# shenwei356/bio

Hardware: AMD Instinct MI355X
Metric: Gbases/s hashed (k=21 ntHash + minimizer) (higher is better)
Workload: dtype u64

## Files before the change

bio_amd/csrc/kernels_pk.hpp:

```cpp
#pragma once
#include <utility>

#include "kernels_fast.hpp"

namespace bsk {

template <int... Is, class F>
__device__ __forceinline__ void pk_unroll_impl(std::integer_sequence<int, Is...>, F &&f) {
    (f(std::integral_constant<int, Is>{}), ...);
}
template <int N, class F>
__device__ __forceinline__ void pk_unroll(F &&f) {
    pk_unroll_impl(std::make_integer_sequence<int, N>{}, f);
}
template <int LO, int HI, class F>
__device__ __forceinline__ void pk_pick(u32 v, F &&f) {
    if constexpr (LO == HI) {
        f(std::integral_constant<int, LO>{});
    } else {
        constexpr int MID = (LO + HI) / 2;
        if (v <= (u32)MID) pk_pick<LO, MID>(v, f);
        else pk_pick<MID + 1, HI>(v, f);
    }
}

#ifndef BSK_PK_ROWS
#define BSK_PK_ROWS 58
#endif
struct PkLds {
    static constexpr int PR = BSK_PK_ROWS;
    static constexpr int ROW = 33;
    static constexpr int TAB = 0;
    static constexpr int TAB2 = 320;
    static constexpr int NHEADS = (32 * (PR - 1)) / 64 + 2;
    static constexpr int HEADS = 0;
    static constexpr int CTAB = 256;
    static constexpr int SH = 768;
    static constexpr int SP = SH + (PR + 1) * ROW * 8;
    static constexpr int TOTAL = (SP + (PR + 1) * ROW * 2 + 15) & ~15;
    static_assert(NHEADS * 8 <= CTAB && CTAB + 512 <= SH && TAB2 + 256 <= SH && TOTAL <= 20480, "PkLds");
};

struct PkTabs {
    u32x4 row;
    u32 at;
    __device__ __forceinline__ void init(int k, int lane, u32 tab = (u32)PkLds::TAB, u32 tab2 = (u32)PkLds::TAB2) {
        row = (u32x4){0, 0, 0, 0};
        at = 0xffffffffu;
        if (lane < 20) {
            const unsigned out = (unsigned)lane >> 2, in = (unsigned)lane & 3u;
            u64 f = seed_fwd_code(in);
            u64 r = rol64(seed_rev_code(in), (unsigned)(k - 1));
            if (out < 4) {
                f ^= rol64(seed_fwd_code(out), (unsigned)k);
                r ^= ror64(seed_rev_code(out), 1);
            }
            row = (u32x4){(u32)f, (u32)(f >> 32), (u32)r, (u32)(r >> 32)};
            at = tab + (u32)lane * 16u;
        } else if (lane >= 32 && lane < 48) {
            const unsigned c0 = (unsigned)lane & 3u, c1 = ((unsigned)lane >> 2) & 3u;
            const u64 f = rol64(seed_fwd_code(c0), 1) ^ seed_fwd_code(c1);
            const u64 r = ror64(rol64(seed_rev_code(c0), (unsigned)(k - 1)), 1) ^ rol64(seed_rev_code(c1), (unsigned)(k - 1));
            row = (u32x4){(u32)f, (u32)(f >> 32), (u32)r, (u32)(r >> 32)};
            at = tab2 + (u32)(lane - 32) * 16u;
        }
    }
    __device__ __forceinline__ void write(LDSQ char *ldsq) const {
        if (at != 0xffffffffu) *reinterpret_cast<LDSQ u32x4 *>(ldsq + at) = row;
        wave_sync_lds();
    }
};

template <int W>
struct PkCfg {
    static constexpr int XC = W > 12 ? 4 : W;
};

#define PKNW 16
typedef u32 u32x16 __attribute__((ext_vector_type(16)));
struct PkWords {
    u32x4 a, b, c, d;
};
__device__ __forceinline__ PkWords pk_load_words(const u32 *p) {
    PkWords r;
    asm volatile("global_load_dwordx4 %0, %4, off\n\tglobal_load_dwordx4 %1, %4, off offset:16\n\t"
                 "global_load_dwordx4 %2, %4, off offset:32\n\tglobal_load_dwordx4 %3, %4, off offset:48"
                 : "=&v"(r.a), "=&v"(r.b), "=&v"(r.c), "=&v"(r.d)
                 : "v"(p));
    return r;
}
__device__ __forceinline__ PkWords pk_load_words_n(const u32 *p, u32 nq) {
    PkWords r;
    asm volatile("global_load_dwordx4 %0, %4, off\n\t"
                 "s_cmp_lt_u32 %5, 3\n\ts_cbranch_scc1 .Lpkw_low%=\n\t"
                 "global_load_dwordx4 %1, %4, off offset:16\n\tglobal_load_dwordx4 %2, %4, off offset:32\n\t"
                 "s_cmp_lt_u32 %5, 4\n\ts_cbranch_scc1 .Lpkw_end%=\n\t"
                 "global_load_dwordx4 %3, %4, off offset:48\n\ts_branch .Lpkw_end%=\n"
                 ".Lpkw_low%=:\n\t"
                 "s_cmp_lt_u32 %5, 2\n\ts_cbranch_scc1 .Lpkw_end%=\n\t"
                 "global_load_dwordx4 %1, %4, off offset:16\n"
                 ".Lpkw_end%=:"
                 : "=&v"(r.a), "=&v"(r.b), "=&v"(r.c), "=&v"(r.d)
                 : "v"(p), "s"(nq)
                 : "scc");
    return r;
}
__device__ __forceinline__ u64 pk_load_u64(const u64 *p) {
    u64 r;
    asm volatile("global_load_dwordx2 %0, %1, off" : "=&v"(r) : "v"(p));
    return r;
}
__device__ __forceinline__ void pk_wait_loads(u64 &d0, u64 &d1) { asm volatile("s_waitcnt vmcnt(0)" : "+v"(d0), "+v"(d1)::"memory"); }
__device__ __forceinline__ void pk_wait_loads(PkWords &p) { asm volatile("s_waitcnt vmcnt(0)" : "+v"(p.a), "+v"(p.b), "+v"(p.c), "+v"(p.d)::"memory"); }
__device__ __forceinline__ void pk_ticket_async(u32 *ticket, u32 &t) {
    u64 ex;
    asm volatile("s_mov_b64 %1, exec\n\ts_mov_b64 exec, 1\n\tglobal_atomic_add %0, %2, %3, off sc0\n\ts_mov_b64 exec, %1"
                 : "+v"(t), "=&s"(ex)
                 : "v"(ticket), "v"(1u)
                 : "memory");
}
__device__ __forceinline__ void pk_wait_loads(PkWords &p, u64 &d0, u32 &f, u32 &t) {
    asm volatile("s_waitcnt vmcnt(0)" : "+v"(p.a), "+v"(p.b), "+v"(p.c), "+v"(p.d), "+v"(d0), "+v"(f), "+v"(t)::"memory");
}
__device__ __forceinline__ void pk_wait_loads(PkWords &p, u32 &f, u32 &t) {
    asm volatile("s_waitcnt vmcnt(0)" : "+v"(p.a), "+v"(p.b), "+v"(p.c), "+v"(p.d), "+v"(f), "+v"(t)::"memory");
}
__device__ __forceinline__ u32 pk_load_u8(const u8 *p) {
    u32 r;
    asm volatile("global_load_ubyte %0, %1, off" : "=&v"(r) : "v"(p));
    return r;
}
template <int W, bool LONG, class LY_ = PkLds, bool RINGM = false, bool SELM = false>
struct PkMin {
    typedef LY_ LY;
    const u32 *__restrict__ w;
    LDSQ char *lds;
    int k, lane;
    u32 nk;
    u32 fl, fh_, rl, rh_;
    u32 S[W];
    u64 H[W];
    u32 SB[W];
    u32 P, bm, tmin;
    u32 nsel;
    u32 slot, spare;
    u32 glo, gspan;
    u32 c8000;
    int sstep;
    u32 send;
    u32 in_lo, in_hi, out_lo, out_hi;
    u32x4 pw;
    u32x16 wr;
    static constexpr bool POS2 = !RINGM && !SELM;
    u32 i2;
    u32 nk_top;

    __device__ __forceinline__ void set_words(const PkWords &p) {
        wr = (u32x16){p.a.x, p.a.y, p.a.z, p.a.w, p.b.x, p.b.y, p.b.z, p.b.w, p.c.x, p.c.y, p.c.z, p.c.w, p.d.x, p.d.y, p.d.z, p.d.w};
    }
    __device__ __forceinline__ void word2(u32 i, u32 &lo, u32 &hi) const {
        const u32 iu = (u32)__builtin_amdgcn_readfirstlane((int)i);
        if (!LONG || iu + 1 < (u32)PKNW) {
            lo = wr[iu], hi = wr[iu + 1];
        } else {
            lo = w[iu], hi = w[iu + 1];
        }
    }
    __device__ __forceinline__ u32 word(u32 i) const {
        const u32 iu = (u32)__builtin_amdgcn_readfirstlane((int)i);
        if constexpr (RINGM) {
            if (iu < 4u) return iu == 0 ? pw.x : iu == 1 ? pw.y : iu == 2 ? pw.z : pw.w;
            return w[iu];
        }
        if (!LONG || iu < (u32)PKNW) return wr[iu];
        return w[iu];
    }
    __device__ __forceinline__ void load_block_words(u32 i0) {
        const u32 t0 = i0 + (u32)k - 1, p0 = i0 - 1;
        in_lo = w[t0 >> 4];
        in_hi = w[(t0 >> 4) + 1];
        out_lo = w[p0 >> 4];
        out_hi = w[(p0 >> 4) + 1];
    }
    __device__ __forceinline__ void load_block0_words() {
        const u32 t0 = (u32)k - 1;
        in_lo = word(t0 >> 4);
        in_hi = word((t0 >> 4) + 1);
        out_lo = word(0);
        out_hi = word(1);
    }
    __device__ __forceinline__ void roll(u32x4 x) {
        const u32 a = __builtin_amdgcn_alignbit(fl, fh_, 31), b = __builtin_amdgcn_alignbit(fh_, fl, 31);
        const u32 c = __builtin_amdgcn_alignbit(rh_, rl, 1), d = __builtin_amdgcn_alignbit(rl, rh_, 1);
        fl = a ^ x.x;
        fh_ = b ^ x.y;
        rl = c ^ x.z;
        rh_ = d ^ x.w;
    }
    __device__ __forceinline__ void roll2(u32x4 x) {
        const u32 a = __builtin_amdgcn_alignbit(fl, fh_, 30), b = __builtin_amdgcn_alignbit(fh_, fl, 30);
        const u32 c = __builtin_amdgcn_alignbit(rh_, rl, 2), d = __builtin_amdgcn_alignbit(rl, rh_, 2);
        fl = a ^ x.x;
        fh_ = b ^ x.y;
        rl = c ^ x.z;
        rh_ = d ^ x.w;
    }

    __device__ __forceinline__ void guard() {
        if constexpr (RINGM || SELM) return;
        const bool in = slot - glo <= gspan;
        slot = in ? slot : spare;
        sstep = in ? sstep : 0;
    }
    template <int IDX, int O>
    __device__ __forceinline__ void emit(u32 pbase) {
        if constexpr (!SELM) emit_staged<IDX, O>(pbase);
    }
    template <int IDX, int O>
    __device__ __forceinline__ void emit_staged(u32 pbase) {
        const u32 b = (bm >> IDX) & 1u;
        u32 pv;
        if constexpr (POS2) {
            (void)pbase;
            pv = SB[O];
        } else {
            asm("v_add3_u32 %0, %1, %2, %3" : "=v"(pv) : "v"(SB[O]), "s"(pbase), "n"(O));
        }
#if defined(PK_MASKST)
        {
            const u32 a0 = (u32)(uintptr_t)(lds + LY::SH) + slot, a1 = (u32)(uintptr_t)(lds + LY::SP) + (slot >> 2);
            u64 sv;
            asm volatile("v_cmp_ne_u32_e32 vcc, 0, %1\n\ts_and_saveexec_b64 %0, vcc\n\tds_write_b64 %2, %3\n\tds_write_b16 %4, %5\n\ts_mov_b64 exec, %0"
                         : "=&s"(sv) : "v"(b), "v"(a0), "v"(H[O]), "v"(a1), "v"(pv) : "vcc", "memory");
        }
#elif defined(PK_NOPOS)
        *reinterpret_cast<LDSQ u64 *>(lds + LY::SH + slot) = H[O];
#ifdef PK_STRMASK
        asm volatile("" ::"v"(pv));
#endif
#elif !defined(PK_NOSTAGE)
        *reinterpret_cast<LDSQ u64 *>(lds + LY::SH + slot) = H[O];
        *reinterpret_cast<LDSQ u16 *>(lds + LY::SP + (slot >> 2)) = (u16)pv;
#else
        asm volatile("" ::"v"(H[O]), "v"(pv), "v"(slot));
#endif
        asm("v_mad_i32_i24 %0, %1, %2, %0" : "+v"(slot) : "v"(b), "v"(sstep));
        if constexpr (RINGM) slot = slot == send ? (u32)lane * 8u : slot;
    }

    template <bool FIRST, bool RAG, int PAR>
    __device__ __forceinline__ void block(u32 i0, u32 okbit, bool suffix) {
        static_assert(!POS2, "POS2 (k_minimizer_pk): i2 is advanced by run()");
        const u32 t0 = i0 + (u32)k - 1, p0 = FIRST ? 0u : i0 - 1u;
        steps<FIRST, RAG, PAR>(2u * t0, 2u * p0, i0, okbit);
        if (suffix) suffix_pass();
        tail<FIRST, PAR>(i0);
    }

    template <bool FIRST, bool RAG, int PAR>
    __device__ __forceinline__ void steps(u32 t2, u32 p2, u32 i0, u32 okbit) {
        constexpr int CB = PAR * 16, PB = (1 - PAR) * 16;
        constexpr int XC = PkCfg<W>::XC;
        constexpr int O2 = PAR ? 0 : 2 * W;
        u32 in_lo, in_hi, out_lo, out_hi;
        if constexpr (RINGM) {
            in_lo = this->in_lo, in_hi = this->in_hi, out_lo = this->out_lo, out_hi = this->out_hi;
            load_block_words(i0 + (u32)W);
        } else {
            word2(t2 >> 5, in_lo, in_hi);
            word2(p2 >> 5, out_lo, out_hi);
        }
        const u32 cinb = __builtin_amdgcn_alignbit(in_hi, in_lo, t2 & 31u);
        u32 coutb;
        if (FIRST) coutb = out_lo << 2;
        else coutb = __builtin_amdgcn_alignbit(out_hi, out_lo, p2 & 31u);
        const u32 E = (cinb & 0x33333333u) | ((coutb & 0x33333333u) << 2);
        const u32 O = ((cinb >> 2) & 0x33333333u) | (coutb & 0xCCCCCCCCu);
        const u32 E4 = E << 4, O4 = O << 4;
        u32x4 xs[W];
        auto fetch = [&](int o0) {
#pragma unroll
            for (int o = o0; o < o0 + XC && o < W; ++o) {
                const int j = o >> 1;
                const u32 src = (j & 1) ? ((o & 1) ? O : E) : ((o & 1) ? O4 : E4);
                u32 a;
                switch (j >> 1) {
                    case 0: asm("v_and_b32_sdwa %0, %1, %2 dst_sel:DWORD dst_unused:UNUSED_PAD src0_sel:BYTE_0 src1_sel:DWORD" : "=v"(a) : "v"(src), "s"(0xF0u)); break;
                    case 1: asm("v_and_b32_sdwa %0, %1, %2 dst_sel:DWORD dst_unused:UNUSED_PAD src0_sel:BYTE_1 src1_sel:DWORD" : "=v"(a) : "v"(src), "s"(0xF0u)); break;
                    case 2: asm("v_and_b32_sdwa %0, %1, %2 dst_sel:DWORD dst_unused:UNUSED_PAD src0_sel:BYTE_2 src1_sel:DWORD" : "=v"(a) : "v"(src), "s"(0xF0u)); break;
                    default: asm("v_and_b32_sdwa %0, %1, %2 dst_sel:DWORD dst_unused:UNUSED_PAD src0_sel:BYTE_3 src1_sel:DWORD" : "=v"(a) : "v"(src), "s"(0xF0u)); break;
                }
                if (FIRST && o == 0) a = 0x100u | (a & 0x30u);
#ifndef PK_NOTAB
                xs[o] = *reinterpret_cast<LDSQ const u32x4 *>(lds + LY::TAB + a);
#else
                xs[o] = (u32x4){a, a ^ E, a + O, a ^ cinb};
#endif
            }
        };
        fetch(0);
        if (XC < W) fetch(XC);
        u32 pbase = 0;
        if constexpr (!POS2) pbase = (u32)__builtin_amdgcn_readfirstlane((int)(i0 - (u32)W));
        if (!FIRST) guard();
        u32 vb = 0;
        if (RAG && !FIRST) {
            const int left = (int)nk - (int)i0;
            const u32 nv = (u32)(left < 0 ? 0 : left > W ? W : left);
            vb = (1u << nv) - 1u;
        }
        constexpr bool CUTB = RAG && !FIRST;
        u32 live = (u32)W;
        if constexpr (CUTB) {
            const u32 left = nk_top - i0;
            live = (u32)__builtin_amdgcn_readfirstlane((int)(left < (u32)W ? left : (u32)W));
        }
        pk_unroll<W>([&](auto oc) {
            constexpr int o = decltype(oc)::value;
            if (XC < W && o && o % XC == 0 && o + XC < W) {
                __builtin_amdgcn_sched_barrier(0);
                fetch(o + XC);
            }
            if constexpr (CUTB) {
                this->template emit<PB + o, o>(pbase);
                if (o != 0 && (u32)o >= live) return;
            }
            roll(xs[o]);
            if constexpr (!CUTB) {
                if (!FIRST) this->template emit<PB + o, o>(pbase);
            }
            const lmask rev = lt64(rl, rh_, fl, fh_);
            const u32 hl = sel(rev, rl, fl), hh = sel(rev, rh_, fh_);
            if constexpr (POS2) {
                lmask co;
                asm("v_addc_co_u32_e64 %0, %1, %2, %3, %4" : "=v"(SB[o]), "=s"(co) : "n"(O2 + 2 * o), "v"(i2), "s"(rev));
            } else {
                asm("v_cndmask_b32_e64 %0, 0, %1, %2" : "=v"(SB[o]) : "v"(c8000), "s"(rev));
            }
            H[o] = ((u64)hh << 32) | hl;
            u32 pk;
            asm("v_and_or_b32 %0, %1, %2, %3" : "=v"(pk) : "v"(hh), "s"(0xffffffe0u), "n"(CB + o));
            if (o == 0) {
                P = pk;
            } else {
#ifndef PK_NOTIE
                const u32 d = pk ^ P;
                tmin = tmin < d ? tmin : d;
#endif
                P = P < pk ? P : pk;
            }
            if (!FIRST || o == W - 1) {
                u32 m = P;
                if constexpr (o != W - 1) {
#ifndef PK_NOTIE
                    const u32 d = P ^ S[o + 1];
                    tmin = tmin < d ? tmin : d;
#endif
                    m = P < S[o + 1] ? P : S[o + 1];
                }
                u32 one = 1u;
                if (FIRST) one = okbit;
                else if (RAG) one = (vb >> o) & 1u;
                bm |= one << (m & 31u);
            }
            S[o] = pk;
        });
    }

    __device__ __forceinline__ void suffix_pass() {
#pragma unroll
        for (int q = W - 2; q >= 1; --q) {
#ifndef PK_NOTIE
            const u32 d = S[q] ^ S[q + 1];
            tmin = tmin < d ? tmin : d;
#endif
            S[q] = S[q] < S[q + 1] ? S[q] : S[q + 1];
        }
    }

    template <bool FIRST, int PAR>
    __device__ __forceinline__ void tail(u32 i0) {
        constexpr int PB = (1 - PAR) * 16;
        if constexpr (SELM) {
            if (!FIRST) {
                const u32 wsel = (bm >> PB) & ((1u << W) - 1u);
                *reinterpret_cast<LDSQ u32 *>(lds + LY::MASK + (i0 / (u32)W - 1u) * 256u + (u32)lane * 4u) = wsel;
                nsel += (u32)__builtin_popcount(wsel);
            }
        }
        if (!FIRST) asm("v_and_b32_e32 %0, %1, %0" : "+v"(bm) : "n"(PAR ? 0xffff0000u : 0x0000ffffu));
    }

    template <int PAR, int O>
    __device__ __forceinline__ void drain_from(u32 pbase, u32 live) {
        if constexpr (O < W) {
            if (O == 0 || (u32)O < live) {
                this->template emit<PAR * 16 + O, O>(pbase);
                drain_from<PAR, O + 1>(pbase, live);
            }
        }
    }

    template <int PAR>
    __device__ __forceinline__ void drain(u32 i0, u32 live = (u32)W) {
        if constexpr (SELM) {
            const u32 wsel = (bm >> (PAR * 16)) & ((1u << W) - 1u);
            *reinterpret_cast<LDSQ u32 *>(lds + LY::MASK + (i0 / (u32)W) * 256u + (u32)lane * 4u) = wsel;
            nsel += (u32)__builtin_popcount(wsel);
            return;
        }
        const u32 pbase = (u32)__builtin_amdgcn_readfirstlane((int)i0);
        guard();
        drain_from<PAR, 0>(pbase, live);
    }

    __device__ __forceinline__ void begin(u32 slot0, int step, u32 col8) {
        fl = fh_ = rl = rh_ = 0;
        bm = 0;
        nsel = 0;
        nk_top = 0xffffffffu;
        c8000 = 0x8000u;
        asm volatile("" : "+v"(c8000));
        tmin = 0xffffffffu;
        slot = slot0;
        sstep = step;
        if constexpr (RINGM) {
            (void)col8;
            spare = glo = gspan = 0;
            send = (u32)(LY::ROWS * LY::ROW * 8) + (u32)lane * 8u;
        } else {
            spare = (u32)(LY::PR * LY::ROW * 8) + col8;
            send = 0;
            constexpr u32 RB = (u32)(LY::ROW * 8);
            glo = step < 0 ? col8 + (u32)(W - 1) * RB : col8;
            gspan = (u32)(LY::PR - W) * RB + (step < 0 ? 0u : RB);
        }
        if constexpr (RINGM) load_block0_words();
        for (int t0 = 0; t0 < k - 1; t0 += 16) {
            const u32 word = this->word((u32)t0 >> 4);
            const int nb = (k - 1 - t0) < 16 ? (k - 1 - t0) : 16;
            int j = 0;
            for (; j + 8 <= nb; j += 8) {
                const u32 sub = word >> (2 * j);
                const u32x4 x0 = *reinterpret_cast<LDSQ const u32x4 *>(lds + LY::TAB2 + ((sub & 0xf) << 4));
                const u32x4 x1 = *reinterpret_cast<LDSQ const u32x4 *>(lds + LY::TAB2 + (sub & 0xf0));
                const u32x4 x2 = *reinterpret_cast<LDSQ const u32x4 *>(lds + LY::TAB2 + ((sub & 0xf00) >> 4));
                const u32x4 x3 = *reinterpret_cast<LDSQ const u32x4 *>(lds + LY::TAB2 + ((sub & 0xf000) >> 8));
                roll2(x0);
                roll2(x1);
                roll2(x2);
                roll2(x3);
            }
            for (; j + 2 <= nb; j += 2) roll2(*reinterpret_cast<LDSQ const u32x4 *>(lds + LY::TAB2 + (((word >> (2 * j)) & 0xf) << 4)));
            for (; j < nb; ++j) roll(*reinterpret_cast<LDSQ const u32x4 *>(lds + LY::TAB + 256 + (((word >> (2 * j)) & 3) << 4)));
        }
    }

    static constexpr bool CARRY = !SELM;
    __device__ __forceinline__ void advance(u32 &i0, u32 &t2, u32 &p2) const {
        if constexpr (CARRY) {
            t2 += 2u * W, p2 += 2u * W;
            asm volatile("" : "+s"(t2), "+s"(p2));
            i0 = (p2 >> 1) + 1u;
        } else {
            i0 += W;
            t2 = 2u * (i0 + (u32)k - 1u), p2 = 2u * (i0 - 1u);
        }
    }

    __device__ __forceinline__ void run(u32 nk_max, bool ok, u32 nk_min, u32 slot0, int step, u32 col8) {
        begin(slot0, step, col8);
        nk_top = nk_max;
        if constexpr (POS2) i2 = (u32)(-2 * W);
        steps<true, false, 0>(2u * ((u32)k - 1u), 0u, 0u, ok ? 1u : 0u);
        if (nk_max <= (u32)W) {
            drain<0>(0);
            return;
        }
        suffix_pass();
        u32 i0 = W;
        u32 t2 = 2u * ((u32)W + (u32)k - 1u), p2 = 2u * ((u32)W - 1u);
        if constexpr (CARRY) asm volatile("" : "+s"(t2), "+s"(p2));
        const int lim = 2 * ((int)__builtin_amdgcn_readfirstlane((int)(nk_min < 0x8000u ? nk_min : 0x8000u)) - 2 * W - 1);
        while ((int)p2 < lim) {
            if constexpr (POS2) asm("v_add_u32_e32 %0, %1, %0" : "+v"(i2) : "n"(4 * W));
            steps<false, false, 1>(t2, p2, i0, 1u);
            suffix_pass();
            tail<false, 1>(i0);
            advance(i0, t2, p2);
            steps<false, false, 0>(t2, p2, i0, 1u);
            suffix_pass();
            tail<false, 0>(i0);
            advance(i0, t2, p2);
        }
        int last_par;
        for (;;) {
            if constexpr (POS2) asm("v_add_u32_e32 %0, %1, %0" : "+v"(i2) : "n"(4 * W));
            steps<false, true, 1>(t2, p2, i0, 1u);
            tail<false, 1>(i0);
            advance(i0, t2, p2);
            last_par = 1;
            if (i0 >= nk_max) break;
            suffix_pass();
            steps<false, true, 0>(t2, p2, i0, 1u);
            tail<false, 0>(i0);
            advance(i0, t2, p2);
            last_par = 0;
            if (i0 >= nk_max) break;
            suffix_pass();
        }
        const u32 left = nk_max - (i0 - (u32)W);
        const u32 live = (u32)__builtin_amdgcn_readfirstlane((int)(left < (u32)W ? left : (u32)W));
        if (last_par) drain<1>(i0 - W, live);
        else drain<0>(i0 - W, live);
    }
};

template <int U, class LY = PkLds, bool POS2 = false, bool TAILR = false>
__device__ __forceinline__ void pk_copyout(char *lds, int lane, u32 cnt, u32 excl, u32 T, u64 base, const KArgs &a) {
    constexpr int NH = LY::NHEADS;
    u64 *s_heads = reinterpret_cast<u64 *>(lds + LY::HEADS);
    u64 *s_tab64 = reinterpret_cast<u64 *>(lds + LY::CTAB);
    const u64 nzmask = __builtin_amdgcn_ballot_w64(cnt > 0);
    if (lane < NH) s_heads[lane] = 0;
    wave_sync_lds();
    if (cnt > 0) {
        constexpr int RB = LY::ROW * 8;
        const int col8 = (lane & 31) * 8;
        const int S = lane < 32 ? RB : -RB;
        const int A = lane < 32 ? col8 - (int)excl * RB : col8 + ((int)(LY::PR - 1) + (int)excl) * RB;
        const u32 rk = __builtin_amdgcn_mbcnt_hi((u32)(nzmask >> 32), __builtin_amdgcn_mbcnt_lo((u32)nzmask, 0));
        s_tab64[rk] = ((u64)(u32)S << 32) | (u32)A;
        if (excl) atomicOr(&s_heads[(excl - 1u) >> 6], 1ULL << ((excl - 1u) & 63u));
    }
    wave_sync_lds();
    const u64 hw = lane < NH ? s_heads[lane] : 0ULL;
    const u32 hw_lo = (u32)hw, hw_hi = (u32)(hw >> 32);
    u32 heads_before = 0;
    const char *sh = lds + LY::SH, *sp = lds + LY::SP;
    u64 *const gh = a.hash + base;
    u32 *const gp = a.pos + base;
    auto trip = [&](u32 t0, auto rows, auto check) {
        constexpr int R = decltype(rows)::value;
        constexpr bool CHECK = decltype(check)::value;
        u32 rank[R];
#pragma unroll
        for (int j = 0; j < R; ++j) {
            const u32 c = (t0 >> 6) + j;
            const u32 mlo = (u32)__builtin_amdgcn_readlane((int)hw_lo, (int)c), mhi = (u32)__builtin_amdgcn_readlane((int)hw_hi, (int)c);
            rank[j] = (__builtin_amdgcn_mbcnt_hi(mhi, __builtin_amdgcn_mbcnt_lo(mlo, 0u)) << 3) + (heads_before << 3);
            heads_before += (u32)__builtin_popcountll(((u64)mhi << 32) | mlo);
        }
        u64 ent[U];
#pragma unroll
        for (int j = 0; j < R; ++j) ent[j] = *reinterpret_cast<const u64 *>(reinterpret_cast<const char *>(s_tab64) + rank[j]);
#pragma unroll
        for (int j = R; j < U; ++j) ent[j] = ent[R - 1];
        if constexpr (U == 8) {
            __builtin_amdgcn_sched_barrier(0);
            asm volatile("" ::"v"(ent[0]), "v"(ent[1]), "v"(ent[2]), "v"(ent[3]), "v"(ent[4]), "v"(ent[5]), "v"(ent[6]), "v"(ent[7]));
            __builtin_amdgcn_sched_barrier(0);
        }
        u64 hv[U];
        u32 pv[U];
#pragma unroll
        for (int j = 0; j < R; ++j) {
            const u32 t = t0 + 64 * j + lane;
            const int off = __mul24((int)t, (int)(u32)(ent[j] >> 32)) + (int)(u32)ent[j];
            const u32 so = (!CHECK || (TAILR && j < R - 1) || t < T) ? (u32)off : 0u;
            hv[j] = *reinterpret_cast<const u64 *>(sh + so);
            if constexpr (POS2) pv[j] = *reinterpret_cast<const u16 *>(sp + (so >> 2));
            else pv[j] = (u32)(int)*reinterpret_cast<const short *>(sp + (so >> 2));
        }
#pragma unroll
        for (int j = R; j < U; ++j) hv[j] = hv[R - 1], pv[j] = pv[R - 1];
        if constexpr (U == 8) {
            __builtin_amdgcn_sched_barrier(0);
            asm volatile("" ::"v"(hv[0]), "v"(hv[1]), "v"(hv[2]), "v"(hv[3]), "v"(hv[4]), "v"(hv[5]), "v"(hv[6]), "v"(hv[7]), "v"(pv[0]), "v"(pv[1]),
                         "v"(pv[2]), "v"(pv[3]), "v"(pv[4]), "v"(pv[5]), "v"(pv[6]), "v"(pv[7]));
            __builtin_amdgcn_sched_barrier(0);
        }
#pragma unroll
        for (int j = 0; j < R; ++j) {
            const u32 t = t0 + 64 * j + lane;
#ifdef PK_NOSTORE
            asm volatile("" ::"v"(hv[j]), "v"(pv[j]));
#else
            if (!CHECK || (TAILR && j < R - 1) || t < T) {
#ifndef PK_NOHASHST
                __builtin_nontemporal_store(hv[j], &gh[t]);
#else
                asm volatile("" ::"v"(hv[j]));
#endif
#ifndef PK_NOPOSST
                __builtin_nontemporal_store(POS2 ? __builtin_amdgcn_alignbit(pv[j], pv[j], 1) : pv[j] & 0x80007fffu, &gp[t]);
#else
                asm volatile("" ::"v"(pv[j]));
#endif
            }
#endif
        }
    };
    u32 t0 = 0;
    for (; t0 + 64 * U <= T; t0 += 64 * U) trip(t0, std::integral_constant<int, U>{}, std::false_type{});
    if (t0 < T) {
        if constexpr (TAILR) {
            const u32 nr = (u32)__builtin_amdgcn_readfirstlane((int)((T - t0 + 63u) >> 6));
            pk_pick<1, U>(nr, [&](auto rc) { trip(t0, rc, std::true_type{}); });
        } else {
            trip(t0, std::integral_constant<int, U>{}, std::true_type{});
        }
    }
    wave_sync_lds();
}

#ifndef PK_TICKET
#define PK_TICKET 8u
#endif
template <int W, bool LONG, bool UNI = false>
__global__ __launch_bounds__(64, 2) void k_minimizer_pk(KArgs a) {
    static_assert(!(UNI && LONG), "k_minimizer_pk: the fixed-length form keeps the whole read in registers");
    typedef PkLds LY;
    __shared__ __attribute__((aligned(16))) char lds[LY::TOTAL];
    LDSQ char *const ldsq = (LDSQ char *)lds;
    const int lane = lane_id();
    PkTabs tabs;
    tabs.init(a.k, lane);
#ifdef PK_STAGGER
    for (u32 i = (((blockIdx.x * 2654435761u) >> 24) * (u32)PK_STAGGER) >> 8; i; --i) __builtin_amdgcn_s_sleep(32);
#endif
    const u64 slab = (u64)64 * BSK_FAST_CAP;
    const u32 col8 = (u32)(lane & 31) * 8u;
    constexpr u32 RB = (u32)(LY::ROW * 8);
    const u32 top = (u32)(LY::PR - 1) * RB + col8;
    u64 d_n1 = 0, d_cur = 0;
    PkWords pw_cur = {{0, 0, 0, 0}, {0, 0, 0, 0}, {0, 0, 0, 0}, {0, 0, 0, 0}};
    bool have = false;
    const u32 lseg = a.fixcap / a.list_grid;
    u32 lcur = 0;
    const u32 tku = a.tk ? a.tk : PK_TICKET;
    const u32 t0s = a.tk_small ? a.tk_t0 : 0xffffffffu, u0s = a.tk_small ? a.tk_t0 * tku : 0xffffffffu;
    const u32 tsm = a.tk_small ? a.tk_small : tku;
    auto ticket_unit = [&](u32 t) { return t < t0s ? t * tku : u0s + (t - t0s) * tsm; };
    auto ticket_end = [&](u32 first) { return first + (first < u0s ? tku : tsm); };
    const u32 uL = a.uniform_len;
    const u32 unk = (UNI && uL >= (u32)a.circ_ext && (uL - (u32)a.circ_ext) + 1u >= (u32)a.k + (u32)W) ? uL - (u32)a.k + 1u : 0u;
    const u32 unq = a.uni_stride / 4u + 1u < 4u ? a.uni_stride / 4u + 1u : 4u;
    const bool ahead = tku >= 3u;
    u32 tv = 0;
    u32 nt = ~0u;
    for (u32 unit = ticket_unit(next_ticket(a.ticket, lane)), uend = ticket_end(unit); unit < a.nunits; ++unit, ({
             if (unit == uend) {
                 unit = ahead ? nt : ticket_unit(next_ticket(a.ticket, lane));
                 uend = ticket_end(unit);
             }
         })) {
        const u64 r = (u64)unit * 64 + lane;
        const u64 u2 = (!ahead || unit + 2u < uend) ? (u64)unit + 2u : (u64)nt + (unit + 2u - uend);
        const bool nxt = unit + 1 != uend ? unit + 1 < a.nunits : ahead && nt < a.nunits;
        const bool ask = ahead && unit + 3u == uend;
        const u64 rmax = a.n - 1;
        if constexpr (UNI) {
            if (!have) {
                pw_cur = pk_load_words_n(a.words + (r < rmax ? r : rmax) * (u64)a.uni_stride, unq);
                pk_wait_loads(pw_cur);
            }
        } else if (!have) {
            d_cur = pk_load_u64(a.desc + (r < rmax ? r : rmax));
            d_n1 = pk_load_u64(a.desc + (r + 64 < rmax ? r + 64 : rmax));
            pk_wait_loads(d_cur, d_n1);
            pw_cur = pk_load_words(a.words + (d_cur >> 24));
            pk_wait_loads(pw_cur);
        }
        PkWords pw_n1;
        u64 d_n2 = 0;
        if constexpr (UNI) {
            const u64 r1 = ((!ahead || unit + 1u < uend) ? (u64)unit + 1u : (u64)nt) * 64 + lane;
            pw_n1 = pk_load_words_n(a.words + (r1 < rmax ? r1 : rmax) * (u64)a.uni_stride, unq);
        } else {
            pw_n1 = pk_load_words(a.words + (d_n1 >> 24));
            const u64 r2 = u2 * 64 + lane;
            d_n2 = pk_load_u64(a.desc + (r2 < rmax ? r2 : rmax));
        }
        u32 rfl = pk_load_u8(a.rflags ? a.rflags + (r < rmax ? r : rmax) : reinterpret_cast<const u8 *>(a.desc));
        if (ask) pk_ticket_async(a.ticket, tv);
        const u64 d = d_cur;
        const PkWords pw = pw_cur;
        u64 off, ro;
        bool ok;
        u32 nk, nk_max, nk_min;
        if constexpr (UNI) {
            off = 0;
            ro = r;
            ok = r < a.n && unk != 0u;
            nk = nk_max = nk_min = unk;
        } else {
            const u64 L = desc_len(a, d);
            off = d >> 24;
            ro = out_index(a, r, d);
            ok = r < a.n && L >= (u64)a.circ_ext && (L - (u64)a.circ_ext) + 1 >= (u64)a.k + (u64)W;
            nk = ok ? (u32)(L - a.k + 1) : 0u;
            nk_max = wave_max_u32(nk);
            nk_min = ~wave_max_u32(~(ok ? nk : 0xffffffffu));
        }
        u32 cnt = 0, tmin_lane = 0xffffffffu;
        if (nk_max) {
            tabs.write(ldsq);
            PkMin<W, LONG> pm;
            pm.w = a.words + off;
            pm.set_words(pw);
            pm.lds = ldsq;
            pm.k = a.k;
            pm.lane = lane;
            pm.nk = nk;
            const u32 spare = (u32)LY::PR * RB + col8;
            pm.run(nk_max, ok, nk_min, !ok ? spare : lane < 32 ? col8 : top, !ok ? 0 : lane < 32 ? (int)RB : -(int)RB, col8);
            if (ok) cnt = (lane < 32 ? pm.slot - col8 : top - pm.slot) / RB;
            tmin_lane = pm.tmin;
        }
        if constexpr (UNI) pk_wait_loads(pw_n1, rfl, tv);
        else pk_wait_loads(pw_n1, d_n2, rfl, tv);
        if (ask) nt = ticket_unit((u32)__builtin_amdgcn_readfirstlane((int)tv));
        d_cur = d_n1;
        pw_cur = pw_n1;
        d_n1 = d_n2;
        have = nxt;
        const u32 cnt_pair = cnt + (u32)__builtin_amdgcn_ds_bpermute((lane ^ 32) * 4, (int)cnt);
        u64 bad = __builtin_amdgcn_ballot_w64(cnt_pair >= (u32)LY::PR);
        u64 tied = __builtin_amdgcn_ballot_w64(ok && tmin_lane < 32u);
#if defined(PK_NOSTAGE) || defined(PK_NOTIE) || defined(PK_NOTAB) || defined(PK_NOCOPY) || defined(PK_NOSTORE) || defined(PK_NOFB)
        bad = 0;
        tied = 0;
#endif
        const u64 redo = bad | tied;
        if (redo) {
            list_append(a, a.rlist, lseg, lcur, redo, lane, r);
            if ((redo >> lane) & 1) cnt = 0;
        }
        const u32 incl = wave_incl_scan_u32(cnt, lane);
        const u32 excl = incl - cnt;
        const u32 T = wave_bcast_u32(incl, 63);
        const u64 base = (u64)unit * slab;
#ifndef PK_NOCOPY
#ifndef PK_CU
#define PK_CU 8
#endif
        if (T) pk_copyout<PK_CU, LY, PkMin<W, LONG>::POS2, true>(lds, lane, cnt, excl, T, base, a);
#endif
        if (r < a.n) {
            if (!((redo >> lane) & 1)) a.refs[ro] = ((base + excl) << 24) | cnt;
            u8 sbyte = ok ? BSK_ST_OK : BSK_ST_SHORT;
            if (ok && a.rflags) sbyte |= (u8)rfl;
            a.status[ro] = sbyte;
        }
    }
    list_close(a.rlist, lseg, lcur, lane);
}

#ifdef BSK_IMPL_PK
#ifndef BSK_PK_WS
#define BSK_PK_WS(X) X(2) X(3) X(4) X(5) X(6) X(7) X(8) X(9) X(10) X(11) X(12) X(13)
#endif
bool pk_minimizer_supported(int w) { return w >= 2 && w <= 13; }
u32 pk_minimizer_short_bases() { return 16u * (PKNW - 1); }
int pk_minimizer_blocks_per_cu(int w) {
    int nb = 0;
    hipError_t e = hipErrorInvalidValue;
    switch (w) {
#define X(WW) \
    case WW: e = hipOccupancyMaxActiveBlocksPerMultiprocessor(&nb, k_minimizer_pk<WW, false>, 64, 0); break;
        BSK_PK_WS(X)
#undef X
        default: break;
    }
    if (e != hipSuccess || nb < 1) {
        (void)hipGetLastError();
        nb = 1;
    }
    return nb;
}
void pk_minimizer_list_launch(int w, int grid, hipStream_t stream, const KArgs &a) {
    switch (w) {
#define X(WW) \
    case WW: hipLaunchKernelGGL((k_minimizer_dense<WW, true>), dim3(grid), dim3(64), 0, stream, a); break;
        BSK_PK_WS(X)
#undef X
        default: break;
    }
}
bool pk_minimizer_uniform(bool long_reads, const KArgs &a) { return !long_reads && a.uni_stride && a.uniform_len && !a.cls_hi && !a.binned && !a.subset; }
void pk_minimizer_launch(int w, bool long_reads, int grid, hipStream_t stream, const KArgs &a) {
    const bool uni = pk_minimizer_uniform(long_reads, a);
    switch (w) {
#define X(WW)                                                                                               \
    case WW:                                                                                                \
        if (long_reads) {                                                                                   \
            hipLaunchKernelGGL((k_minimizer_pk<WW, true>), dim3(grid), dim3(64), 0, stream, a);             \
        } else if (uni) {                                                                                   \
            hipLaunchKernelGGL((k_minimizer_pk<WW, false, true>), dim3(grid), dim3(64), 0, stream, a);      \
        } else {                                                                                            \
            hipLaunchKernelGGL((k_minimizer_pk<WW, false>), dim3(grid), dim3(64), 0, stream, a);            \
        }                                                                                                   \
        hipLaunchKernelGGL((k_minimizer_dense<WW, true>), dim3(grid), dim3(64), 0, stream, a);              \
        break;
        BSK_PK_WS(X)
#undef X
        default: break;
    }
}
#endif

}
```

bio_amd/csrc/kernels_ring.hpp:

```cpp
#pragma once
#include "kernels_pk.hpp"
#pragma clang diagnostic ignored "-Winline-asm"

namespace bsk {

typedef u32 u32x3 __attribute__((ext_vector_type(3)));
#ifdef RG_B96
typedef u32x3 u32x3_lds __attribute__((aligned(16)));
#else
typedef u32x3 u32x3_lds __attribute__((aligned(4)));
#endif

#ifndef BSK_RING_WAVES
#define BSK_RING_WAVES 3
#endif
#ifndef BSK_RING_NQ
#define BSK_RING_NQ (BSK_RING_WAVES >= 3 ? 3 : 4)
#endif
#ifndef BSK_RING_EVERY
#define BSK_RING_EVERY 1
#endif
#ifndef BSK_RING_FIRST
#define BSK_RING_FIRST 4
#endif
// ... 282 lines not shown
#else
        asm volatile("" ::"v"(HL[O]), "v"(HH[O]), "v"(pv), "v"(at));
#endif
        asm("v_lshl_add_u32 %0, %1, 28, %0" : "+v"(phase) : "v"(b));
    }

    template <bool FIRST, bool RAG, int PAR>
    __device__ __forceinline__ void block(u32 i0, u32 okbit, bool suffix) {
        constexpr int CB = PAR * 16, PB = (1 - PAR) * 16;
        constexpr int XC = RgCfg<W>::XC;
        const u32 t0 = i0 + (u32)k - 1, p0 = FIRST ? 0u : i0 - 1u;
        u32 in_lo, in_hi, out_lo, out_hi;
        this->template word2<PAR>(t0 >> 4, true, in_lo, in_hi);
        this->template word2<PAR>(p0 >> 4, false, out_lo, out_hi);
        const u32 cinb = __builtin_amdgcn_alignbit(in_hi, in_lo, (t0 & 15) * 2);
        u32 coutb;
        if (FIRST) coutb = out_lo << 2;
        else coutb = __builtin_amdgcn_alignbit(out_hi, out_lo, (p0 & 15) * 2);
        const u32 E = (cinb & 0x33333333u) | ((coutb & 0x33333333u) << 2);
        const u32 O = ((cinb >> 2) & 0x33333333u) | (coutb & 0xCCCCCCCCu);
        const u32 E4 = E << 4, O4 = O << 4;
        u32x4 xs[W];
        auto fetch = [&](int o0) {
#pragma unroll
            for (int o = o0; o < o0 + XC && o < W; ++o) {
                const int j = o >> 1;
                const u32 src = (j & 1) ? ((o & 1) ? O : E) : ((o & 1) ? O4 : E4);
                u32 a;
                switch (j >> 1) {
                    case 0: asm("v_and_b32_sdwa %0, %1, %2 dst_sel:DWORD dst_unused:UNUSED_PAD src0_sel:BYTE_0 src1_sel:DWORD" : "=v"(a) : "v"(src), "s"(0xF0u)); break;
                    case 1: asm("v_and_b32_sdwa %0, %1, %2 dst_sel:DWORD dst_unused:UNUSED_PAD src0_sel:BYTE_1 src1_sel:DWORD" : "=v"(a) : "v"(src), "s"(0xF0u)); break;
                    case 2: asm("v_and_b32_sdwa %0, %1, %2 dst_sel:DWORD dst_unused:UNUSED_PAD src0_sel:BYTE_2 src1_sel:DWORD" : "=v"(a) : "v"(src), "s"(0xF0u)); break;
                    default: asm("v_and_b32_sdwa %0, %1, %2 dst_sel:DWORD dst_unused:UNUSED_PAD src0_sel:BYTE_3 src1_sel:DWORD" : "=v"(a) : "v"(src), "s"(0xF0u)); break;
                }
                if (FIRST && o == 0) a = 0x100u | (a & 0x30u);
                xs[o] = *reinterpret_cast<LDSQ const u32x4 *>(lds + LY::TAB + a);
            }
        };
        fetch(0);
        if (XC < W) fetch(XC);
        u32 pbase = 2u * (i0 - (u32)W);
        asm volatile("" : "+v"(pbase));
        u32 vb = 0;
        if (RAG && !FIRST) {
            const int left = (int)nk - (int)i0;
            const u32 nv = (u32)(left < 0 ? 0 : left > W ? W : left);
            vb = (1u << nv) - 1u;
        }
        pk_unroll<W>([&](auto oc) {
            constexpr int o = decltype(oc)::value;
            if (XC < W && o && o % XC == 0 && o + XC < W) {
                __builtin_amdgcn_sched_barrier(0);
                fetch(o + XC);
            }
            roll(xs[o]);
            const lmask rev = lt64(rl, rh_, fl, fh_);
            if (!FIRST) this->template emit<PB + o, o>(pbase);
            const u32 hl = sel(rev, rl, fl), hh = sel(rev, rh_, fh_);
            HL[o] = hl;
            HH[o] = hh;
            RV[o] = rev;
            u32 pk;
            asm("v_and_or_b32 %0, %1, %2, %3" : "=v"(pk) : "v"(hh), "s"(0xffffffe0u), "n"(CB + o));
            if (o == 0) {
                P = pk;
            } else {
#ifndef RG_NOTIE
                const u32 d = pk ^ P;
                tmin = tmin < d ? tmin : d;
#endif
                P = P < pk ? P : pk;
            }
            if (!FIRST || o == W - 1) {
                u32 m = P;
                if constexpr (o != W - 1) {
#ifndef RG_NOTIE
                    const u32 d = P ^ S[o + 1];
                    tmin = tmin < d ? tmin : d;
#endif
                    m = P < S[o + 1] ? P : S[o + 1];
                }
                u32 one = 1u;
                if (FIRST) one = okbit;
                else if (RAG) one = (vb >> o) & 1u;
                bm |= one << (m & 31u);
            }
            S[o] = pk;
        });
        if (suffix) {
#pragma unroll
            for (int q = W - 2; q >= 0; --q) {
#ifndef RG_NOTIE
                const u32 d = S[q] ^ S[q + 1];
                tmin = tmin < d ? tmin : d;
#endif
                S[q] = S[q] < S[q + 1] ? S[q] : S[q + 1];
            }
        }
        if (!FIRST) {
            c += (u32)__builtin_popcount(bm & (PAR ? 0x0000ffffu : 0xffff0000u));
            bm &= PAR ? 0xffff0000u : 0x0000ffffu;
        }
    }

    template <int PAR>
    __device__ __forceinline__ void drain(u32 i0) {
        u32 pbase = 2u * i0;
        asm volatile("" : "+v"(pbase));
        pk_unroll<W>([&](auto oc) {
            constexpr int o = decltype(oc)::value;
            this->template emit<PAR * 16 + o, o>(pbase);
        });
        c += (u32)__builtin_popcount(bm);
    }

    __device__ __forceinline__ void begin() {
        fl = fh_ = rl = rh_ = 0;
        bm = 0;
        c = 0;
        tmin = 0xffffffffu;
        phase = ((u32)lane * (1u << 22) + 2u) / 3u;
        for (int t0 = 0; t0 < k - 1; t0 += 16) {
            const u32 word = this->word((u32)t0 >> 4);
            const int nb = (k - 1 - t0) < 16 ? (k - 1 - t0) : 16;
            int j = 0;
            for (; j + 8 <= nb; j += 8) {
                const u32 sub = word >> (2 * j);
                const u32x4 x0 = *reinterpret_cast<LDSQ const u32x4 *>(lds + LY::TAB2 + ((sub & 0xf) << 4));
                const u32x4 x1 = *reinterpret_cast<LDSQ const u32x4 *>(lds + LY::TAB2 + (sub & 0xf0));
                const u32x4 x2 = *reinterpret_cast<LDSQ const u32x4 *>(lds + LY::TAB2 + ((sub & 0xf00) >> 4));
                const u32x4 x3 = *reinterpret_cast<LDSQ const u32x4 *>(lds + LY::TAB2 + ((sub & 0xf000) >> 8));
                roll2(x0);
                roll2(x1);
                roll2(x2);
                roll2(x3);
            }
            for (; j + 2 <= nb; j += 2) roll2(*reinterpret_cast<LDSQ const u32x4 *>(lds + LY::TAB2 + (((word >> (2 * j)) & 0xf) << 4)));
            for (; j < nb; ++j) roll(*reinterpret_cast<LDSQ const u32x4 *>(lds + LY::TAB + 256 + (((word >> (2 * j)) & 3) << 4)));
        }
    }
};

#ifndef RG_TICKET
#define RG_TICKET 8u
#endif
template <int W, int NQ, bool LONG>
__global__ __launch_bounds__(64, BSK_RING_WAVES) RG_KERNEL_ATTR void k_minimizer_ring(KArgs a) {
    typedef RgLds LY;
    __shared__ __attribute__((aligned(16))) char lds[LY::TOTAL];
    LDSQ char *const ldsq = (LDSQ char *)lds;
    const int lane = lane_id();
    {
        PkTabs tabs;
        tabs.init(a.k, lane);
        tabs.write(ldsq);
    }
#ifdef RG_STAGGER
    for (u32 i = (((blockIdx.x * 2654435761u) >> 24) * (u32)RG_STAGGER) >> 8; i; --i) __builtin_amdgcn_s_sleep(32);
#endif
    const u32 rows = a.unit_rows;
    const u64 slab = (u64)64 * rows;
    const bool uniform_batch = a.uniform_len != 0;
    const u32 lane4 = (u32)lane * 4u, lane8 = (u32)lane * 8u;
    u64 d_n1 = 0, d_cur = 0;
    RgWords<NQ> pw_cur;
#pragma unroll
    for (int j = 0; j < NQ; ++j) pw_cur.q[j] = (u32x4){0, 0, 0, 0};
    bool have = false;
    const u32 lseg = a.fixcap / a.list_grid;
    u32 lcur = 0;
    const u32 tku = a.tk ? a.tk : RG_TICKET;
    for (u32 unit = next_ticket(a.ticket, lane) * tku, uend = unit + tku; unit < a.nunits; ++unit, ({
             if (unit == uend) {
                 unit = next_ticket(a.ticket, lane) * tku;
                 uend = unit + tku;
             }
         })) {
        const u64 r = (u64)unit * 64 + lane;
        const bool nxt = unit + 1 != uend && unit + 1 < a.nunits;
        const u64 rmax = a.n - 1;
        if (!have) {
            d_cur = pk_load_u64(a.desc + (r < rmax ? r : rmax));
            d_n1 = pk_load_u64(a.desc + (r + 64 < rmax ? r + 64 : rmax));
            pk_wait_loads(d_cur, d_n1);
            pw_cur = rg_load_words<NQ>(a.words + (d_cur >> 24));
            rg_wait_loads<NQ>(pw_cur);
        }
#if BSK_RING_WAVES >= 3
        rg_prefetch_issue(a.words + (d_n1 >> 24), a.desc + (r + 128 < rmax ? r + 128 : rmax),
                          a.rflags ? a.rflags + (r < rmax ? r : rmax) : reinterpret_cast<const u8 *>(a.desc));
#else
        RgWords<NQ> pw_n1 = rg_load_words<NQ>(a.words + (d_n1 >> 24));
        u64 d_n2 = pk_load_u64(a.desc + (r + 128 < rmax ? r + 128 : rmax));
        u32 rfl = pk_load_u8(a.rflags ? a.rflags + (r < rmax ? r : rmax) : reinterpret_cast<const u8 *>(a.desc));
#endif
        const u64 d = d_cur;
        const u64 off = d >> 24, L = desc_len(a, d);
        const u64 ro = out_index(a, r, d);
        const bool ok = r < a.n && L >= (u64)a.circ_ext && (L - (u64)a.circ_ext) + 1 >= (u64)a.k + (u64)W;
        const u32 nk = ok ? (u32)(L - a.k + 1) : 0u;
        const u32 nk_max = wave_max_u32(nk);
        const bool uniform = uniform_batch && __builtin_amdgcn_ballot_w64(ok) == ~0ULL;
#if defined(RG_L2STORE) || defined(RG_SMALLSLAB)
        const u64 base = (u64)blockIdx.x * slab;
#else
        const u64 base = (u64)unit * slab;
#endif
        const u64 *const sh = a.hash + base;
        const u32 *const sp = a.pos + base;
        RgMin<W, NQ, LONG> pm;
        pm.w = a.words + off;
        pm.set_words(pw_cur);
        pm.lds = ldsq;
        pm.k = a.k;
        pm.lane = lane;
        pm.nk = nk;
        u32 T = 0, g = 0;
        lmask lost = 0;
        auto group = [&](u32 tg, auto mode, int hi, int lo) {
            const u32 va = lane4 + (tg & (u32)(LY::R - 1)) * (u32)LY::ROWB;
#ifdef RG_SMALLSLAB
            rg_group<decltype(mode)::value>(va, lane8 + (tg & 4u) * 512u, lane4 + (tg & 4u) * 256u, sh, sp, hi, lo);
#else
            rg_group<decltype(mode)::value>(va, lane8 + tg * 512u, lane4 + tg * 256u, sh, sp, hi, lo);
#endif
        };
        auto catch_up = [&](u32 top, u32 lazy) {
            if (!__builtin_amdgcn_ballot_w64(top - g >= lazy)) return;
            const lmask need = __builtin_amdgcn_ballot_w64(g < top);
            for (u32 tg = T - (u32)LY::G;; tg -= (u32)LY::G) {
                const lmask here = need & __builtin_amdgcn_ballot_w64(g < tg + (u32)LY::G);
                if (here & __builtin_amdgcn_ballot_w64(top > tg)) group(tg, std::integral_constant<int, 2>{}, (int)(top - tg), (int)(g - tg));
                if (!(here & __builtin_amdgcn_ballot_w64(g < tg)) || tg == 0) break;
            }
            g = top;
        };
        auto round = [&](u32 i0_done) {
            lost |= __builtin_amdgcn_ballot_w64(pm.c - g >= (u32)LY::R);
            catch_up(pm.c < T ? pm.c : T, (u32)LY::LAZY);
            const bool lagging = g < T;
            const lmask lag = __builtin_amdgcn_ballot_w64(lagging);
            const lmask act = uniform ? ~0ULL : __builtin_amdgcn_ballot_w64(pm.nk > i0_done);
            for (;;) {
                if (T + (u32)LY::G > rows) break;
                const lmask behind = act & __builtin_amdgcn_ballot_w64(pm.c < T + (u32)LY::G);
                if (behind && !__builtin_amdgcn_ballot_w64(pm.c >= T + (u32)(LONG ? LY::PRESS_LONG : LY::PRESS_SHORT))) break;
                if (!behind && !lag && uniform) group(T, std::integral_constant<int, 0>{}, 0, 0);
                else group(T, std::integral_constant<int, 1>{}, lagging ? 0 : (int)(pm.c - T), 0);
                T += (u32)LY::G;
            }
            g = lagging ? g : (pm.c < T ? pm.c : T);
        };
        pm.begin();
        pm.template block<true, false, 0>(0, ok ? 1u : 0u, nk_max > (u32)W);
#if BSK_RING_WAVES < 3
        rg_wait_loads<NQ>(pw_n1, d_n2, rfl);
#endif
        u32 i0 = W;
        int last_par = 0;
        u32 nround = 0;
        pm.template issue_next<1>(W);
        pm.template issue_next<0>(2 * W);
        for (;;) {
            if (i0 >= nk_max) break;
            {
                const bool more = i0 + W < nk_max;
                if (uniform && i0 + W <= nk_max) pm.template block<false, false, 1>(i0, 1u, more);
                else pm.template block<false, true, 1>(i0, 1u, more);
            }
            i0 += W;
            last_par = 1;
            if (i0 >= nk_max) break;
            pm.wait_next();
            ++nround;
#if BSK_RING_WAVES >= 3
            if (nround == BSK_RING_FIRST) rg_prefetch_wait();
#endif
            if (nround >= BSK_RING_FIRST) round(i0 - W);
            pm.template issue_next<1>(i0 + W);
            {
                const bool more = i0 + W < nk_max;
                if (uniform && i0 + W <= nk_max) pm.template block<false, false, 0>(i0, 1u, more);
                else pm.template block<false, true, 0>(i0, 1u, more);
            }
            i0 += W;
            last_par = 0;
            if (i0 >= nk_max) break;
            pm.wait_next();
            ++nround;
#if BSK_RING_WAVES >= 3
            if (nround == BSK_RING_FIRST) rg_prefetch_wait();
#endif
            if (nround >= BSK_RING_FIRST) round(i0 - W);
            pm.template issue_next<0>(i0 + W);
        }
#if BSK_RING_WAVES >= 3
        if (nround < BSK_RING_FIRST) rg_prefetch_wait();
#endif
        if (last_par) pm.template drain<1>(i0 - W);
        else pm.template drain<0>(i0 - W);
        const u32 cnt = ok ? pm.c : 0u;
        const u32 lim = cnt < rows ? cnt : rows;
        lost |= __builtin_amdgcn_ballot_w64(cnt - g >= (u32)LY::R);
        u64 redo = __builtin_amdgcn_ballot_w64(ok && (pm.tmin < 32u || cnt > rows)) | (lost & __builtin_amdgcn_ballot_w64(ok));
#if defined(RG_NOSTAGE) || defined(RG_NOTIE) || defined(RG_NOSTORE) || defined(RG_NOFB)
        redo = 0;
#endif
// ... 70 lines not shown
```

Before: 1310.

## Warm up ntHash with 3-base LDS table and clamp staging slot via med3

Adds a 64-entry, 3-base combined ntHash table in LDS so the k-1 warm-up bases are absorbed three at a time (roll3), in groups of four lookups, instead of two at a time. The out-of-range staging guard is replaced by a single v_med3 clamp on the slot. Overflow detection moves to a post-run count check that forces the redo path. This shortens the serial warm-up dependency chain and the per-drain guard cost, but adds a table write per unit into the staging area and changes the overflow semantics.

```diff
diff --git a/bio_amd/csrc/kernels_pk.hpp b/bio_amd/csrc/kernels_pk.hpp
--- a/bio_amd/csrc/kernels_pk.hpp
+++ b/bio_amd/csrc/kernels_pk.hpp
@@ -31,20 +31,20 @@
     static constexpr int PR = BSK_PK_ROWS;
     static constexpr int ROW = 33;
     static constexpr int TAB = 0;
-    static constexpr int TAB2 = 320;
     static constexpr int NHEADS = (32 * (PR - 1)) / 64 + 2;
     static constexpr int HEADS = 0;
     static constexpr int CTAB = 256;
     static constexpr int SH = 768;
     static constexpr int SP = SH + (PR + 1) * ROW * 8;
     static constexpr int TOTAL = (SP + (PR + 1) * ROW * 2 + 15) & ~15;
-    static_assert(NHEADS * 8 <= CTAB && CTAB + 512 <= SH && TAB2 + 256 <= SH && TOTAL <= 20480, "PkLds");
+    static constexpr int TAB3 = SH;
+    static_assert(NHEADS * 8 <= CTAB && CTAB + 512 <= SH && TAB + 320 <= SH && TAB3 % 16 == 0 && TAB3 + 1024 <= SP && TOTAL <= 20480, "PkLds");
 };
 
 struct PkTabs {
     u32x4 row;
     u32 at;
-    __device__ __forceinline__ void init(int k, int lane, u32 tab = (u32)PkLds::TAB, u32 tab2 = (u32)PkLds::TAB2) {
+    __device__ __forceinline__ void init(int k, int lane, u32 tab, u32 tab2) {
         row = (u32x4){0, 0, 0, 0};
         at = 0xffffffffu;
         if (lane < 20) {
@@ -57,7 +57,7 @@
             }
             row = (u32x4){(u32)f, (u32)(f >> 32), (u32)r, (u32)(r >> 32)};
             at = tab + (u32)lane * 16u;
-        } else if (lane >= 32 && lane < 48) {
+        } else if (tab2 != 0xffffffffu && lane >= 32 && lane < 48) {
             const unsigned c0 = (unsigned)lane & 3u, c1 = ((unsigned)lane >> 2) & 3u;
             const u64 f = rol64(seed_fwd_code(c0), 1) ^ seed_fwd_code(c1);
             const u64 r = ror64(rol64(seed_rev_code(c0), (unsigned)(k - 1)), 1) ^ rol64(seed_rev_code(c1), (unsigned)(k - 1));
@@ -68,6 +68,21 @@
     __device__ __forceinline__ void write(LDSQ char *ldsq) const {
         if (at != 0xffffffffu) *reinterpret_cast<LDSQ u32x4 *>(ldsq + at) = row;
         wave_sync_lds();
+    }
+};
+
+struct PkTab3 {
+    u32x4 row;
+    __device__ __forceinline__ void init(int k, int lane) {
+        const unsigned c0 = (unsigned)lane & 3u, c1 = ((unsigned)lane >> 2) & 3u, c2 = ((unsigned)lane >> 4) & 3u;
+        const u64 r0 = rol64(seed_rev_code(c0), (unsigned)(k - 1)), r1 = rol64(seed_rev_code(c1), (unsigned)(k - 1)), r2 = rol64(seed_rev_code(c2), (unsigned)(k - 1));
+        const u64 f = rol64(seed_fwd_code(c0), 2) ^ rol64(seed_fwd_code(c1), 1) ^ seed_fwd_code(c2);
+        const u64 r = ror64(r0, 2) ^ ror64(r1, 1) ^ r2;
+        row = (u32x4){(u32)f, (u32)(f >> 32), (u32)r, (u32)(r >> 32)};
+    }
+    template <class LY>
+    __device__ __forceinline__ void write(LDSQ char *ldsq, int lane) const {
+        *reinterpret_cast<LDSQ u32x4 *>(ldsq + LY::TAB3 + lane * 16) = row;
     }
 };
 
@@ -143,8 +158,8 @@
     u32 SB[W];
     u32 P, bm, tmin;
     u32 nsel;
-    u32 slot, spare;
-    u32 glo, gspan;
+    u32 slot;
+    u32 glo, ghi;
     u32 c8000;
     int sstep;
     u32 send;
@@ -152,6 +167,7 @@
     u32x4 pw;
     u32x16 wr;
     static constexpr bool POS2 = !RINGM && !SELM;
+    static constexpr bool WARM3 = !RINGM && !SELM;
     u32 i2;
     u32 nk_top;
 
@@ -205,12 +221,18 @@
         rl = c ^ x.z;
         rh_ = d ^ x.w;
     }
+    __device__ __forceinline__ void roll3(u32x4 x) {
+        const u32 a = __builtin_amdgcn_alignbit(fl, fh_, 29), b = __builtin_amdgcn_alignbit(fh_, fl, 29);
+        const u32 c = __builtin_amdgcn_alignbit(rh_, rl, 3), d = __builtin_amdgcn_alignbit(rl, rh_, 3);
+        fl = a ^ x.x;
+        fh_ = b ^ x.y;
+        rl = c ^ x.z;
+        rh_ = d ^ x.w;
+    }
 
     __device__ __forceinline__ void guard() {
         if constexpr (RINGM || SELM) return;
-        const bool in = slot - glo <= gspan;
-        slot = in ? slot : spare;
-        sstep = in ? sstep : 0;
+        asm("v_med3_i32 %0, %0, %1, %2" : "+v"(slot) : "v"(glo), "v"(ghi));
     }
     template <int IDX, int O>
     __device__ __forceinline__ void emit(u32 pbase) {
@@ -414,6 +436,48 @@
         drain_from<PAR, 0>(pbase, live);
     }
 
+    __device__ __forceinline__ void warm3() {
+        const u32 nb = (u32)k - 1u, ng = nb / 3u;
+        auto window = [&](u32 bit) {
+            u32 lo, hi;
+            word2(bit >> 5, lo, hi);
+            return __builtin_amdgcn_alignbit(hi, lo, bit & 31u);
+        };
+        auto row3 = [&](u32 a) { return *reinterpret_cast<LDSQ const u32x4 *>(lds + LY::TAB3 + (a & 0x3f0u)); };
+        auto row1 = [&](u32 a) { return *reinterpret_cast<LDSQ const u32x4 *>(lds + LY::TAB + 256 + (a & 0x30u)); };
+        auto four = [&](u32 g, auto first) {
+            const u32 sub = window(6u * g);
+            const u32x4 x0 = row3(sub << 4), x1 = row3(sub >> 2), x2 = row3(sub >> 8), x3 = row3(sub >> 14);
+            __builtin_amdgcn_sched_barrier(0);
+            asm volatile("" ::"v"(x0), "v"(x1), "v"(x2), "v"(x3));
+            __builtin_amdgcn_sched_barrier(0);
+            if constexpr (decltype(first)::value) fl = x0.x, fh_ = x0.y, rl = x0.z, rh_ = x0.w;
+            else roll3(x0);
+            roll3(x1);
+            roll3(x2);
+            roll3(x3);
+        };
+        u32 g = 0;
+        if (ng >= 4u) {
+            four(0u, std::true_type{});
+            for (g = 4u; g + 4u <= ng; g += 4u) four(g, std::false_type{});
+        }
+        const u32 gl = ng - g, sl = nb - 3u * ng;
+        if (gl | sl) {
+            const u32 sub = window(6u * g);
+            const u32 one = sub >> (6u * gl);
+            const u32x4 x0 = row3(sub << 4), x1 = row3(sub >> 2), x2 = row3(sub >> 8), y0 = row1(one << 4), y1 = row1(one << 2);
+            __builtin_amdgcn_sched_barrier(0);
+            asm volatile("" ::"v"(x0), "v"(x1), "v"(x2), "v"(y0), "v"(y1));
+            __builtin_amdgcn_sched_barrier(0);
+            if (gl >= 1u) roll3(x0);
+            if (gl >= 2u) roll3(x1);
+            if (gl >= 3u) roll3(x2);
+            if (sl >= 1u) roll(y0);
+            if (sl >= 2u) roll(y1);
+        }
+    }
+
     __device__ __forceinline__ void begin(u32 slot0, int step, u32 col8) {
         fl = fh_ = rl = rh_ = 0;
         bm = 0;
@@ -426,16 +490,20 @@
         sstep = step;
         if constexpr (RINGM) {
             (void)col8;
-            spare = glo = gspan = 0;
+            glo = ghi = 0;
             send = (u32)(LY::ROWS * LY::ROW * 8) + (u32)lane * 8u;
         } else {
-            spare = (u32)(LY::PR * LY::ROW * 8) + col8;
             send = 0;
             constexpr u32 RB = (u32)(LY::ROW * 8);
-            glo = step < 0 ? col8 + (u32)(W - 1) * RB : col8;
-            gspan = (u32)(LY::PR - W) * RB + (step < 0 ? 0u : RB);
+            static_assert(SELM || LY::PR >= 2 * W, "PkMin: the guard's bounds");
+            glo = step < 0 ? col8 + (u32)(W - 1) * RB : step > 0 ? col8 : slot0;
+            ghi = step < 0 ? col8 + (u32)(LY::PR - 1) * RB : step > 0 ? col8 + (u32)(LY::PR - W + 1) * RB : slot0;
         }
         if constexpr (RINGM) load_block0_words();
+        if constexpr (WARM3) warm3();
+        else warm2();
+    }
+    __device__ __forceinline__ void warm2() {
         for (int t0 = 0; t0 < k - 1; t0 += 16) {
             const u32 word = this->word((u32)t0 >> 4);
             const int nb = (k - 1 - t0) < 16 ? (k - 1 - t0) : 16;
@@ -625,7 +693,9 @@
     LDSQ char *const ldsq = (LDSQ char *)lds;
     const int lane = lane_id();
     PkTabs tabs;
-    tabs.init(a.k, lane);
+    tabs.init(a.k, lane, (u32)LY::TAB, 0xffffffffu);
+    PkTab3 tab3;
+    tab3.init(a.k, lane);
 #ifdef PK_STAGGER
     for (u32 i = (((blockIdx.x * 2654435761u) >> 24) * (u32)PK_STAGGER) >> 8; i; --i) __builtin_amdgcn_s_sleep(32);
 #endif
@@ -703,8 +773,9 @@
             nk_max = wave_max_u32(nk);
             nk_min = ~wave_max_u32(~(ok ? nk : 0xffffffffu));
         }
-        u32 cnt = 0, tmin_lane = 0xffffffffu;
+        u32 cnt = 0, cnt_over = 0, tmin_lane = 0xffffffffu;
         if (nk_max) {
+            tab3.write<LY>(ldsq, lane);
             tabs.write(ldsq);
             PkMin<W, LONG> pm;
             pm.w = a.words + off;
@@ -716,6 +787,7 @@
             const u32 spare = (u32)LY::PR * RB + col8;
             pm.run(nk_max, ok, nk_min, !ok ? spare : lane < 32 ? col8 : top, !ok ? 0 : lane < 32 ? (int)RB : -(int)RB, col8);
             if (ok) cnt = (lane < 32 ? pm.slot - col8 : top - pm.slot) / RB;
+            if (cnt >= (u32)(lane < 32 ? LY::PR - W + 1 : LY::PR - W)) cnt_over = (u32)LY::PR;
             tmin_lane = pm.tmin;
         }
         if constexpr (UNI) pk_wait_loads(pw_n1, rfl, tv);
@@ -725,7 +797,8 @@
         pw_cur = pw_n1;
         d_n1 = d_n2;
         have = nxt;
-        const u32 cnt_pair = cnt + (u32)__builtin_amdgcn_ds_bpermute((lane ^ 32) * 4, (int)cnt);
+        const u32 cnt_g = cnt + cnt_over;
+        const u32 cnt_pair = cnt_g + (u32)__builtin_amdgcn_ds_bpermute((lane ^ 32) * 4, (int)cnt_g);
         u64 bad = __builtin_amdgcn_ballot_w64(cnt_pair >= (u32)LY::PR);
         u64 tied = __builtin_amdgcn_ballot_w64(ok && tmin_lane < 32u);
 #if defined(PK_NOSTAGE) || defined(PK_NOTIE) || defined(PK_NOTAB) || defined(PK_NOCOPY) || defined(PK_NOSTORE) || defined(PK_NOFB)
diff --git a/bio_amd/csrc/kernels_ring.hpp b/bio_amd/csrc/kernels_ring.hpp
--- a/bio_amd/csrc/kernels_ring.hpp
+++ b/bio_amd/csrc/kernels_ring.hpp
@@ -458,7 +458,7 @@
     const int lane = lane_id();
     {
         PkTabs tabs;
-        tabs.init(a.k, lane);
+        tabs.init(a.k, lane, (u32)LY::TAB, (u32)LY::TAB2);
         tabs.write(ldsq);
     }
 #ifdef RG_STAGGER
```

Result: no change. 1317, median of 6 (+0.5%).
